# ConwayBeyond/Funscript-Flow

Hardware: AMD Instinct MI355X
Metric: 1080p frame-pairs/sec (higher is better)
Workload: dtype f32

## Files before the change

funscript_flow_amd/csrc/ffl_api.hip:

```cpp
#include "../../include/ffl.h"
#include "ffl_kernels.h"

#include <math.h>
#include <stdarg.h>
#include <stdio.h>
#include <string.h>

#include <algorithm>
#include <condition_variable>
#include <mutex>
#include <string>
#include <thread>
#include <vector>

#define FFL_EV_RING 16
#define FFL_RAW_RING 4

template <class H, class Arg, hipError_t (*Free)(Arg)>
struct Owned {
    H h = H();
    Owned() = default;
    explicit Owned(H take) : h(take) {}
    Owned(Owned &&o) noexcept : h(o.release()) {}
    Owned &operator=(Owned &&o) noexcept { std::swap(h, o.h); return *this; }
// ... 27 lines not shown
    hipError_t create(int n) {
        ev = std::vector<Event>(n);
        for (auto &e : ev) {
            hipError_t r = hipEventCreateWithFlags(e.put(), hipEventDisableTiming);
            if (r != hipSuccess) return r;
        }
        return hipSuccess;
    }
    hipError_t settle_next() {
        if (next < ev.size() || next < settled) return hipSuccess;
        const hipError_t r = hipEventSynchronize(ev[next % ev.size()]);
        if (r == hipSuccess) settled = next + 1;
        return r;
    }
    hipError_t record(hipStream_t st, EvRef *out);
};
struct EvRef {
    const EvRing *ring = nullptr;
    unsigned long long ticket = 0;
    hipEvent_t get() const { return (ring && ring->next - ticket <= ring->ev.size()) ? ring->ev[ticket % ring->ev.size()].h : nullptr; }
};
inline hipError_t EvRing::record(hipStream_t st, EvRef *out) {
    hipError_t r = settle_next();
    if (r == hipSuccess) r = hipEventRecord(ev[next % ev.size()], st);
    if (r == hipSuccess) *out = EvRef{this, next++};
    return r;
}
static inline EvRef ev_latest(const EvRing &r) { return r.next ? EvRef{&r, r.next - 1} : EvRef{}; }

struct ProfRec {
    int cls;
    hipEvent_t a, b;
    bool shared_start;
};

struct LevelGeom {
    int lw, lh, ksize;
    double sigma;
    GaussKernel gk;
};
struct Geometry { int levels = 0; LevelGeom lv[8]; };

struct Layout {
    size_t i_off[8], t_off[8], r_off[8];
    size_t I, T, R;
    size_t M, flow;
    size_t p1, tab;
    size_t gray, bgr;
    size_t slots, res;
};

struct CopyPool {
    struct Job {
        uint8_t *dst;
        const uint8_t *const *srcs;
        size_t row_bytes, dst_frame;
        ptrdiff_t src_pitch;
        int rows, g0, g1;
    };
    std::vector<std::thread> workers;
    std::mutex mu;
    std::condition_variable cv_work, cv_done;
    std::vector<Job> jobs;
    std::vector<char> busy;
    bool stop = false;

// ... 322 lines not shown
    level_geometry(w, h, &geo);
    const size_t N = (size_t)w * h, maxU = 2 * (size_t)max_batch;
    Layout l = {};
    for (int k = 0; k <= geo.levels; k++) {
        const size_t plane = (size_t)geo.lv[k].lw * geo.lv[k].lh;
        l.i_off[k] = l.I; l.t_off[k] = l.T; l.r_off[k] = l.R;
        l.I += plane * maxU;
        l.T += ffl_pyr_tmp_floats(w, h, geo.lv[k].lw) * maxU;
        l.R += 5 * plane * maxU;
    }
    l.M = 5 * N * max_batch; l.flow = 2 * N * max_batch;
    l.p1 = (size_t)ffl_pass1_blocks(w, h) * max_batch; l.tab = FFL_EV_RING;
    l.gray = (size_t)n_frame_slots * N; l.bgr = (size_t)n_frame_slots * N * 3;
    l.slots = 2 * N * n_flow_slots; l.res = n_flow_slots;
    return l;
}

static hipEvent_t prof_event(ffl_ctx *c) {
    Event e;
    if (c->prof_pool.empty()) {
        hipEventCreate(e.put());
    } else {
        e = std::move(c->prof_pool.back());
        c->prof_pool.pop_back();
    }
    return e.release();
}

struct ProfScope {
    ffl_ctx *c;
    int cls;
    hipEvent_t a = nullptr, b = nullptr;
    bool on, shared = false;
    ProfScope(ffl_ctx *c_, int cls_, hipStream_t st, bool chain = false)
        : c(c_), cls(cls_), on((c_->prof_mask >> cls_) & 1u) {
        if (on) {
            stream = st;
            if (chain && c->prof_last_end && c->prof_last_cls == cls && c->prof_last_stream == st) {
                a = c->prof_last_end;
                shared = true;
            } else {
                a = prof_event(c);
                hipEventRecord(a, st);
            }
        } else {
            c->prof_last_end = nullptr;
        }
    }
    ~ProfScope() {
        if (on) {
            b = prof_event(c);
            hipEventRecord(b, stream);
            c->prof_recs.push_back({cls, a, b, shared});
            c->prof_last_end = b;
            c->prof_last_cls = cls;
            c->prof_last_stream = stream;
        }
    }
    hipStream_t stream = nullptr;
};

static void prof_collect(ffl_ctx *c) {
    for (auto &r : c->prof_recs) {
        float ms = 0;
        hipEventSynchronize(r.b);
        hipEventElapsedTime(&ms, r.a, r.b);
        c->prof_launches[r.cls]++;
        c->prof_ms[r.cls] += ms;
    }
    for (auto &r : c->prof_recs) {
        if (!r.shared_start) c->prof_pool.emplace_back(r.a);
        c->prof_pool.emplace_back(r.b);
    }
    c->prof_recs.clear();
    c->prof_last_end = nullptr;
}

struct WaitOnce {
    hipStream_t st;
    hipEvent_t seen[8];
    int n = 0;
    explicit WaitOnce(hipStream_t s) : st(s) {}
    hipError_t operator()(hipEvent_t e) {
        if (!e) return hipSuccess;
        for (int k = 0; k < n; k++)
            if (seen[k] == e) return hipSuccess;
        if (n < 8) seen[n++] = e;
        return hipStreamWaitEvent(st, e, 0);
    }
};

static int wait_unlocked(ffl_ctx *c, CtxLock &lk, const hipEvent_t *evs, int n) {
    HIPCHK(c, hipSetDevice(c->device));
    lk.unlock();
    hipError_t e = hipSuccess;
    for (int i = 0; i < n && e == hipSuccess; i++)
        if (evs[i]) e = hipEventSynchronize(evs[i]);
    lk.lock();
    if (e != hipSuccess) return set_err(c, FFL_ERR_HIP, "hipEventSynchronize failed: %s", hipGetErrorString(e));
    return FFL_OK;
// ... 685 lines not shown
                                int layout, int depth, int msb_aligned, int rw, int rh, int crop_x, int crop_y,
                                const ffl_source_info *si) {
    return upload_yuv(c, "ffl_upload_frames_yuv16", first, n, (const uint8_t *const *)frames, sw, sh, stride_bytes, layout, 2,
                      depth, msb_aligned != 0, rw, rh, crop_x, crop_y, si);
}

int ffl_upload_frame(ffl_ctx *c, int fslot, const uint8_t *data, int width, int height, int channels,
                     ptrdiff_t stride_bytes) {
    return ffl_upload_frames(c, fslot, 1, &data, width, height, channels, stride_bytes);
}

int ffl_download_frame(ffl_ctx *c, int fslot, uint8_t *dst) {
    if (!c) return FFL_ERR_INVALID;
    CtxLock lk(c->mu);
    if (!dst || fslot < 0 || fslot >= c->n_fslots)
        return set_err(c, FFL_ERR_INVALID, "ffl_download_frame: bad frame slot %d", fslot);
    if (!c->frame_valid[fslot]) return set_err(c, FFL_ERR_STATE, "ffl_download_frame: frame slot %d was never uploaded", fslot);
    HIPCHK(c, hipSetDevice(c->device));
    HIPCHK(c, hipMemcpyAsync(dst, c->d_gray + (size_t)fslot * c->N, c->N, hipMemcpyDeviceToHost, c->s_copy));
    HIPCHK(c, hipStreamSynchronize(c->s_copy));
    return FFL_OK;
}

struct DebugCapture {
    int level, iter;
    float *I0, *I1, *R0, *R1, *M, *flow;
};

static int enqueue_batch(ffl_ctx *c, ffl_ctx::Lane &L, const BatchTab &T, int n, int nU, int pov_mode, const DebugCapture *cap) {
    hipStream_t st = L.st;
    const size_t N = c->N;
    const UTab *ut = &L.d_tab->ut;
    const PairTab *pt = &L.d_tab->pt;
    auto pyr_level = [&](int k, hipStream_t s) { ffl_launch_pyr_level(c->d_gray, N, ut, nU, L.pyr[c->geo.levels - k], s); };
    auto expand_level = [&](int k, hipStream_t s) {
        {
            ProfScope ps(c, FFL_K_PYRAMID, s);
            pyr_level(k, s);
        }
        {
            ProfScope ps(c, FFL_K_POLYEXP, s);
            ffl_launch_polyexp(L.poly[c->geo.levels - k], nU, c->pc, s);
        }
    };
    const int mode = cap ? 0 : c->opt.run_ahead;
    if (mode) {
        for (int k = 0; k < (mode == 2 ? 4 : 1); k++)
            if (!L.st_aux[k]) HIPCHK(c, hipStreamCreateWithFlags(L.st_aux[k].put(), hipStreamNonBlocking));
        HIPCHK(c, hipEventRecord(L.ev_fork, st));
        for (int k = c->geo.levels; k >= 0; k--) {
            hipStream_t sa = L.st_aux[mode == 2 ? k : 0];
            if (mode == 2 || k == c->geo.levels) HIPCHK(c, hipStreamWaitEvent(sa, L.ev_fork, 0));
            expand_level(k, sa);
            HIPCHK(c, hipEventRecord(L.ev_R[k], sa));
        }
        if (mode == 2)
            for (int k = c->geo.levels; k >= 0; k--) HIPCHK(c, hipStreamWaitEvent(st, L.ev_R[k], 0));
    }
    const bool run_ahead = mode == 1;
    bool expanded = mode != 0;
    if (mode == 0 && c->opt.merge_expand) {
        const PyrJob *l0 = &L.pyr[L.n_jobs - 1];
        const bool fuse_l0 = c->opt.fuse_l0_blur && ffl_polyexp_from_gray_ok(*l0);
        const int skip_l0 = fuse_l0 && !cap;
        {
            ProfScope ps(c, FFL_K_PYRAMID, st);
            if (!ffl_launch_pyr_multi(c->d_gray, N, ut, nU, L.pyr, L.n_jobs - skip_l0, c->opt, st))
                for (int k = c->geo.levels; k >= skip_l0; k--) pyr_level(k, st);
        }
        {
            ProfScope ps(c, FFL_K_POLYEXP, st);
            ffl_launch_polyexp_multi(L.poly, L.n_jobs, nU, c->pc, c->d_gray, N, ut, fuse_l0 ? l0 : nullptr, st);
        }
        expanded = true;
    }

    int pw = 0, ph = 0;
    for (int k = c->geo.levels; k >= 0; k--) {
        const LevelGeom &g = c->geo.lv[k];
        const int lw = g.lw, lh = g.lh;
        const size_t plane = (size_t)lw * lh;
        const size_t I_stride = plane, R_stride = 5 * plane, M_stride = 5 * plane;
        float *Rk = L.d_R + c->lay.r_off[k];
        if (pw == 0 && cap)
            for (int i = 0; i < n; i++) HIPCHK(c, hipMemsetAsync(T.pt.flow[k][i], 0, sizeof(float) * 2 * plane, st));
        if (run_ahead) HIPCHK(c, hipStreamWaitEvent(st, L.ev_R[k], 0));
        else if (!expanded) expand_level(k, st);
        int mi = 0;
        const bool fuse_first = c->opt.fuse_first > 0 && !cap && (long)((lw + 63) / 64) * ((lh + 15) / 16) * n >= c->opt.fuse_first;
        if (!fuse_first) {
            ProfScope ps(c, FFL_K_UPDATE_MATRICES, st);
            ffl_launch_update_matrices(Rk, R_stride, plane, pt, k, n, L.d_M[mi], M_stride, lw, lh, pw, ph, pw == 0, cap != nullptr, c->opt, st);
        }
        bool captured = false;
        auto capture = [&]() -> int {
            HIPCHK(c, hipStreamSynchronize(st));
            if (cap->I0) HIPCHK(c, hipMemcpy(cap->I0, L.d_I + c->lay.i_off[k] + (size_t)T.pt.u0[0] * I_stride, sizeof(float) * plane, hipMemcpyDeviceToHost));
            if (cap->I1) HIPCHK(c, hipMemcpy(cap->I1, L.d_I + c->lay.i_off[k] + (size_t)T.pt.u1[0] * I_stride, sizeof(float) * plane, hipMemcpyDeviceToHost));
            if (cap->R0) HIPCHK(c, hipMemcpy(cap->R0, Rk + (size_t)T.pt.u0[0] * R_stride, sizeof(float) * 5 * plane, hipMemcpyDeviceToHost));
            if (cap->R1) HIPCHK(c, hipMemcpy(cap->R1, Rk + (size_t)T.pt.u1[0] * R_stride, sizeof(float) * 5 * plane, hipMemcpyDeviceToHost));
            if (cap->M) HIPCHK(c, hipMemcpy(cap->M, L.d_M[mi], sizeof(float) * 5 * plane, hipMemcpyDeviceToHost));
// ... 1353 lines not shown
```

funscript_flow_amd/csrc/ffl_kernels.h:

```cpp
#pragma once
#include <hip/hip_runtime.h>
#include <limits.h>
#include <stdint.h>

#define FFL_MAXB 256
#define FFL_MAXU (2 * FFL_MAXB)
#define FFL_MAX_LEVELS 4
#define FFL_POLY_N 5
#define FFL_WIN 15
#define FFL_WIN_R 7

struct PolyConsts {
    float g[FFL_POLY_N + 1], xg[FFL_POLY_N + 1], xxg[FFL_POLY_N + 1];
    double gd[FFL_POLY_N + 1], xxgd[FFL_POLY_N + 1];
    double ig11, ig03, ig33, ig55;
};

struct GaussKernel {
    float k[32];
    int ksize;
};

struct UTab {
    int fslot[FFL_MAXU];
// ... 70 lines not shown
    float *tmp, *I;
    size_t tmp_stride, I_stride;
    GaussKernel gk;
};
struct PyrJobs {
    PyrJob j[FFL_MAX_JOBS];
    int n;
};
struct PolyJob {
    const float *I;
    float *R;
    size_t I_stride, R_stride, plane;
    int w, h;
    unsigned gx, gy, first, count;
    int from_gray;
    float gk0, gk1;
};
struct PolyJobs {
    PolyJob j[FFL_MAX_JOBS];
    int n;
};

struct FflOptions {
    int lanes = 2;
    int run_ahead = 0;
    int fuse_first = 10000;
    int merge_expand = 1;
    int use_graph = 1;
    int copy_threads = 4;
    int blur_rows = 0;
    int blur_min_wgs = 3500;
    int tile_order = 0;
    int pyr_coarse = 1;
    int fuse_l0_blur = 1;
    int fb_general = 0;
    int import_fused = 1;
};
struct FflOptionRow {
    const char *name;
    int FflOptions::*member;
    int lo, hi;
    bool flag;
};
inline constexpr FflOptionRow kFflOptionRows[] = {
    {"lanes", &FflOptions::lanes, 1, 4, false},
    {"run_ahead", &FflOptions::run_ahead, 0, 2, false},
    {"fuse_first", &FflOptions::fuse_first, 0, INT_MAX, false},
    {"merge_expand", &FflOptions::merge_expand, INT_MIN, INT_MAX, true},
    {"graph", &FflOptions::use_graph, INT_MIN, INT_MAX, true},
    {"copy_threads", &FflOptions::copy_threads, 1, 16, false},
    {"blur_rows", &FflOptions::blur_rows, 0, 64, false},
    {"blur_min_wgs", &FflOptions::blur_min_wgs, 1, INT_MAX, false},
    {"tile_order", &FflOptions::tile_order, 0, 1, false},
    {"pyr_coarse", &FflOptions::pyr_coarse, INT_MIN, INT_MAX, true},
    {"fuse_l0_blur", &FflOptions::fuse_l0_blur, INT_MIN, INT_MAX, true},
    {"fb_general", &FflOptions::fb_general, 0, 1, false},
    {"import_fused", &FflOptions::import_fused, 0, 1, false},
};

bool ffl_launch_pyr_multi(const uint8_t *gray_base, size_t gray_stride, const UTab *ut, int nU, const PyrJob *levels, int n,
                          const FflOptions &opt, hipStream_t st);
bool ffl_polyexp_from_gray_ok(const PyrJob &l0);
void ffl_launch_polyexp_multi(const PolyJob *levels, int n, int nU, PolyConsts pc, const uint8_t *gray_base, size_t gray_stride,
                              const UTab *ut, const PyrJob *l0, hipStream_t st);
void ffl_launch_frontend(const FrameDesc &d, uint8_t *gray, const FrontParams &p, hipStream_t st);
void ffl_launch_frontend_dev(const FrameDesc *tab, int n, uint8_t *gray_base, size_t N, const FrontParams &p, hipStream_t st);
void ffl_launch_export_flows(const float *flow, const ExportTab &tab, int n, size_t N, char *dst, long long item_stride,
                             int layout, hipStream_t st);
void ffl_launch_import_pass1(const ImportArgs &a, const ExportTab &tab, int n, int dtype, int mode, int w, int h, int pov_mode,
                             int fused, PairTab *pt, unsigned long long *pkey, double *psum, hipStream_t st);
void ffl_launch_gray(const uint8_t *bgr, uint8_t *gray, int n_pixels, hipStream_t st);
size_t ffl_pyr_tmp_floats(int w, int h, int lw);
bool ffl_pyr_level_ok(int w, int h, int lw, int lh, int ksize);
void ffl_launch_pyr_level(const uint8_t *gray_base, size_t gray_stride, const UTab *ut, int nU, const PyrJob &level,
                          hipStream_t st);
void ffl_launch_polyexp(const PolyJob &level, int nU, PolyConsts pc, hipStream_t st);
void ffl_launch_update_matrices(const float *R, size_t R_stride, size_t plane, const PairTab *pt, int level, int nB, float *M,
                                size_t M_stride, int lw, int lh, int pw, int ph, int zero_flow, int store_flow,
                                const FflOptions &opt, hipStream_t st);
void ffl_launch_blur_solve(const float *Min, float *Mout, size_t M_stride, const float *R, size_t R_stride,
                           size_t plane, const PairTab *pt, int level, int nB, int lw, int lh, int update, int store_flow,
                           const FflOptions &opt, hipStream_t st);


void ffl_launch_blur_solve_first(float *Mout, size_t M_stride, const float *R, size_t R_stride, size_t plane,
                                 const PairTab *pt, int level, int nB, int lw, int lh, int pw, int ph, const FflOptions &opt,
                                 hipStream_t st);

#define DIS_MAX_PATCHES 4096
#define DIS_MAX_SCALES 12
struct DisKParams {
    int w, h, finest, coarsest, stride, gd_iters, vr_iters, mean_norm, spatial_prop, stripes;
    float alpha, gamma, delta;
    size_t pair_floats;
    size_t pyr_floats;
    size_t pyr_off[DIS_MAX_SCALES];
    float *dbg;
    int dbg_scale, dbg_stage;
};
void ffl_launch_dis(const UTab *ut, const PairTab *pt, int nB, const uint8_t *gray, size_t gray_stride, float *scratch,
                    const DisKParams &p, hipStream_t st);

int ffl_pass1_blocks(int w, int h);
void ffl_launch_pass1(const PairTab *pt, int nB, int w, int h, int pov_mode, unsigned long long *pkey, double *psum,
                      hipStream_t st);

#define FFL_WINDOW_MAX_RADIUS 32
struct WindowSeq {
// ... 209 lines not shown
```

funscript_flow_amd/csrc/kernels_farneback.hip:

```cpp
#include "ffl_kernels.h"

__global__ __launch_bounds__(256) void k_gray(const uint8_t *__restrict__ bgr, uint8_t *__restrict__ gray, int n) {
    int i4 = (blockIdx.x * 256 + threadIdx.x) * 4;
    if (i4 + 3 < n) {
        const uint32_t *p = reinterpret_cast<const uint32_t *>(bgr + (size_t)i4 * 3);
        uint32_t a = p[0], b = p[1], c = p[2];
        uint32_t px[12] = {a & 255, (a >> 8) & 255, (a >> 16) & 255, a >> 24, b & 255, (b >> 8) & 255,
                           (b >> 16) & 255, b >> 24, c & 255, (c >> 8) & 255, (c >> 16) & 255, c >> 24};
        uint32_t o = 0;
#pragma unroll
        for (int j = 0; j < 4; j++) {
            uint32_t g = (px[j * 3] * 3735u + px[j * 3 + 1] * 19235u + px[j * 3 + 2] * 9798u + 16384u) >> 15;
            o |= g << (8 * j);
        }
        *reinterpret_cast<uint32_t *>(gray + i4) = o;
    } else {
        for (int i = i4; i < n; i++) {
            uint32_t b = bgr[(size_t)i * 3], g = bgr[(size_t)i * 3 + 1], r = bgr[(size_t)i * 3 + 2];
            gray[i] = (uint8_t)((b * 3735u + g * 19235u + r * 9798u + 16384u) >> 15);
        }
    }
}

void ffl_launch_gray(const uint8_t *bgr, uint8_t *gray, int n_pixels, hipStream_t st) {
// ... 132 lines not shown
                v1 = v1 + gk.k[R + j] * (V[c - j].y + V[c + j].y);
            }
            t[qy] = v0 * a0 + (a1 == 0.f ? 0.f : v1) * a1;
        }
    } else {
#pragma unroll
        for (int qy = 0; qy < 2; qy++) {
            if (qy == 1 && b1 == 0.f) break;
            const int cy = qy ? y1 : y0;
            float2 c = col[(size_t)cy * lw];
            float v0 = gk.k[R] * c.x, v1 = gk.k[R] * c.y;
#pragma unroll
            for (int j = 1; j <= R; j++) {
                const float2 m = col[(size_t)ffl_reflect101(cy - j, h) * lw], p = col[(size_t)ffl_reflect101(cy + j, h) * lw];
                v0 = v0 + gk.k[R + j] * (m.x + p.x);
                v1 = v1 + gk.k[R + j] * (m.y + p.y);
            }
            t[qy] = v0 * a0 + (a1 == 0.f ? 0.f : v1) * a1;
        }
    }
    if (dyy < lh) I[(size_t)u * I_stride + (size_t)dy * lw + dx] = t[0] * b0 + t[1] * b1;
}
template <int R>
__global__ __launch_bounds__(256) void k_pyr_v2(const float *__restrict__ tmp, size_t tmp_stride, int w, int h, int lw,
                                                int lh, double sx, double sy, GaussKernel gk, float *__restrict__ I,
                                                size_t I_stride) {
    k_pyr_v2_body<R>(blockIdx.x, blockIdx.y, blockIdx.z, tmp, tmp_stride, w, h, lw, lh, sx, sy, gk, I, I_stride);
}

#ifndef FFL_FR1
#define FFL_FR1 8
#define FFL_FR2 2
#endif
template <int S, int FR, bool ALIGNED>
__device__ __forceinline__ void k_pyr_fused3x4_body(const unsigned bx, const unsigned by, const unsigned bz, const uint8_t *__restrict__ gray_base, size_t gray_stride, const UTab *__restrict__ ut,
                                                      int w, int h, int lw, int lh, GaussKernel gk,
                                                      float *__restrict__ I, size_t I_stride) {
    constexpr int NR = S * FR + 2;
    constexpr int NBY = 4 * S + 2;
    const int dx = 4 * (bx * 256 + threadIdx.x), u = bz;
    if (dx >= lw) return;
    const uint8_t *img = gray_base + (size_t)ut->fslot[u] * gray_stride;
    const int cx = S * dx;
    const bool wide = (ALIGNED || (w & 3) == 0) && cx >= 4 && cx + 4 * S + 4 <= w;
    const float k0 = gk.k[1], k1 = gk.k[2];
    const int dy0 = by * FR;
    float H[NR][4 * S];
#pragma unroll
    for (int j = 0; j < NR; j++) {
        const int sy = ffl_reflect101(min(S * dy0 - 1 + j, h + 1), h);
        const uint8_t *row = img + (size_t)sy * w;
        float b[NBY];
        if (wide) {
            uint32_t wd[S + 2];
            if (S == 1) {
                struct __attribute__((packed, aligned(4))) u3 { uint32_t a, b, c; };
                const u3 t = *reinterpret_cast<const u3 *>(row + cx - 4);
                wd[0] = t.a; wd[1] = t.b; wd[2] = t.c;
            } else {
                struct __attribute__((packed, aligned(4))) u4 { uint32_t a, b, c, d; };
                const u4 t = *reinterpret_cast<const u4 *>(row + cx - 4);
                wd[0] = t.a; wd[1] = t.b; wd[2] = t.c; wd[3] = t.d;
            }
            b[0] = (float)(wd[0] >> 24);
#pragma unroll
            for (int t = 0; t < 4 * S; t++) b[1 + t] = (float)((wd[1 + (t >> 2)] >> (8 * (t & 3))) & 255u);
            b[NBY - 1] = (float)(wd[S + 1] & 255u);
        } else {
#pragma unroll
            for (int t = 0; t < NBY; t++) b[t] = (float)row[ffl_reflect101(cx - 1 + t, w)];
        }
#pragma unroll
        for (int c = 0; c < 4 * S; c++) H[j][c] = ffl_blur3(b[c], b[c + 1], b[c + 2], k0, k1);
    }
#pragma unroll
    for (int o = 0; o < FR; o++) {
        const int dy = dy0 + o;
        if (dy >= lh) break;
        const int c = S * o + 1;
        float out[4];
#pragma unroll
        for (int i = 0; i < 4; i++) {
            if (S == 1) {
                out[i] = ffl_lerp_identity(ffl_blur3(H[c - 1][i], H[c][i], H[c + 1][i], k0, k1));
            } else {
                const float v00 = ffl_blur3(H[c - 1][2 * i], H[c][2 * i], H[c + 1][2 * i], k0, k1);
                const float v01 = ffl_blur3(H[c - 1][2 * i + 1], H[c][2 * i + 1], H[c + 1][2 * i + 1], k0, k1);
                const float v10 = ffl_blur3(H[c][2 * i], H[c + 1][2 * i], H[c + 2][2 * i], k0, k1);
                const float v11 = ffl_blur3(H[c][2 * i + 1], H[c + 1][2 * i + 1], H[c + 2][2 * i + 1], k0, k1);
                const float t0 = v00 * 0.5f + v01 * 0.5f, t1 = v10 * 0.5f + v11 * 0.5f;
                out[i] = t0 * 0.5f + t1 * 0.5f;
            }
        }
        float *dst = I + (size_t)u * I_stride + (size_t)dy * lw + dx;
        if (ALIGNED || dx + 3 < lw) {
            ffl_f4u t;
            t.x = out[0]; t.y = out[1]; t.z = out[2]; t.w = out[3];
            *reinterpret_cast<ffl_f4u *>(dst) = t;
        } else {
#pragma unroll
            for (int i = 0; i < 4; i++)
                if (dx + i < lw) dst[i] = out[i];
        }
    }
}
template <int S, int FR, bool ALIGNED>
__global__ __launch_bounds__(256) void k_pyr_fused3x4(const uint8_t *__restrict__ gray_base, size_t gray_stride, const UTab *__restrict__ ut,
                                                      int w, int h, int lw, int lh, GaussKernel gk,
                                                      float *__restrict__ I, size_t I_stride) {
    k_pyr_fused3x4_body<S, FR, ALIGNED>(blockIdx.x, blockIdx.y, blockIdx.z, gray_base, gray_stride, ut, w, h, lw, lh, gk, I, I_stride);
}

#define PC_TW 128
#define PC_TH 64
#define PC_PW 36
#define PC_PH 76
template <int R, int S>
struct PcLevel {
    static constexpr int NC = PC_TW / S;
    static constexpr int NO = NC * (PC_TH / S);
    static constexpr int HROWS = PC_TH + 2 * R - S + 2;
    static constexpr int HROW0 = S / 2 + 5 - R;
    static constexpr int PITCH = 2 * NC + 2;
    static constexpr int B0 = S / 2 + 7 - R;
    static constexpr int ND = (B0 % 4 + 2 * R + 5) / 4;
    static_assert(HROW0 >= 0 && HROW0 + HROWS <= PC_PH && B0 >= 0 && (NC - 1) * (S / 4) + B0 / 4 + ND <= PC_PW, "tile halo");
};
template <int R, int S>
__device__ __forceinline__ void k_pyr_coarse_h(const uint32_t (*sP)[PC_PW], float (*sH)[PcLevel<R, S>::PITCH], const GaussKernel &gk,
                                               int tid) {
    using L = PcLevel<R, S>;
    constexpr int RSTEP = 256 / L::NC, TRIPS = (L::HROWS + RSTEP - 1) / RSTEP, UNROLL = R == 4 ? 3 : TRIPS;
    constexpr int C = L::B0 % 4 + R;
    const int dl = tid % L::NC, rr = tid / L::NC;
#pragma unroll UNROLL
    for (int k = 0; k < TRIPS; k++) {
        const int ry = rr + RSTEP * k;
// ... 12 lines not shown
            *reinterpret_cast<float2 *>(&sH[ry][2 * dl]) = make_float2(a0, a1);
        }
    }
}
template <int R, int S>
__device__ __forceinline__ void k_pyr_coarse_v(const float (*sH)[PcLevel<R, S>::PITCH], const GaussKernel &gk, int tid, int X0,
                                               int Y0, int w, int h, float *__restrict__ I) {
    using L = PcLevel<R, S>;
    const float a1 = 0.5f, a0 = 1.f - a1, b1 = 0.5f, b0 = 1.f - b1;
    const int lw = w / S, lh = h / S;
#pragma unroll
    for (int k = 0; k < (L::NO + 255) / 256; k++) {
        const int o = tid + 256 * k, el = o / L::NC, dl = o % L::NC;
        if (L::NO % 256 != 0 && o >= L::NO) break;
        const int dx = X0 / S + dl, dy = Y0 / S + el;
        float2 V[2 * R + 2];
#pragma unroll
        for (int j = 0; j < 2 * R + 2; j++) V[j] = *reinterpret_cast<const float2 *>(&sH[S * el + j][2 * dl]);
        float tq[2];
#pragma unroll
        for (int qy = 0; qy < 2; qy++) {
            const int c = R + qy;
            float v0 = gk.k[R] * V[c].x, v1 = gk.k[R] * V[c].y;
#pragma unroll
            for (int j = 1; j <= R; j++) {
                v0 = v0 + gk.k[R + j] * (V[c - j].x + V[c + j].x);
                v1 = v1 + gk.k[R + j] * (V[c - j].y + V[c + j].y);
            }
            tq[qy] = v0 * a0 + v1 * a1;
        }
        if (dx < lw && dy < lh) I[(size_t)dy * lw + dx] = tq[0] * b0 + tq[1] * b1;
    }
}
__global__ __launch_bounds__(256) void k_pyr_coarse(const uint8_t *__restrict__ gray_base, size_t gray_stride,
                                                    const UTab *__restrict__ ut, int w, int h, GaussKernel gk2,
                                                    GaussKernel gk3, float *__restrict__ I2, size_t I2_stride,
                                                    float *__restrict__ I3, size_t I3_stride, int tiles_x, int tiles_y,
                                                    int nU) {
    using L2 = PcLevel<4, 4>;
    using L3 = PcLevel<9, 8>;
    __shared__ __attribute__((aligned(8))) uint32_t sP[PC_PH][PC_PW];
    __shared__ __attribute__((aligned(8))) float sH2[L2::HROWS][L2::PITCH];
    __shared__ __attribute__((aligned(8))) float sH3[L3::HROWS][L3::PITCH];
    const int tid = threadIdx.x;
    const unsigned per = (unsigned)tiles_x * tiles_y;
    unsigned tt;
    if (!ffl_xcd_tile(blockIdx.x, per * nU, tt)) return;
    const int u = tt / per, t = tt - u * per, ty = t / tiles_x, tx = t - ty * tiles_x;
    const int X0 = tx * PC_TW, Y0 = ty * PC_TH;
    const uint8_t *img = gray_base + (size_t)ut->fslot[u] * gray_stride;
    constexpr int PCQ = PC_PW / 4, NLOAD = (PC_PH * PCQ + 255) / 256;
#pragma unroll
    for (int k = 0; k < NLOAD; k++) {
        const int i = tid + 256 * k;
        if (i < PC_PH * PCQ) {
            const int ry = i / PCQ, q = i - ry * PCQ;
            const int gy = ffl_reflect101(Y0 - 6 + ry, h), X = X0 - 8 + 16 * q;
            const uint8_t *row = img + (size_t)gy * w;
            uint32_t v[4];
            ffl_gray16_reflect101(row, X, w, true, v);
            *reinterpret_cast<uint2 *>(&sP[ry][4 * q]) = make_uint2(v[0], v[1]);
            *reinterpret_cast<uint2 *>(&sP[ry][4 * q + 2]) = make_uint2(v[2], v[3]);
        }
    }
    __syncthreads();
    k_pyr_coarse_h<4, 4>(sP, sH2, gk2, tid);
    k_pyr_coarse_h<9, 8>(sP, sH3, gk3, tid);
    __syncthreads();
    k_pyr_coarse_v<4, 4>(sH2, gk2, tid, X0, Y0, w, h, I2 + (size_t)u * I2_stride);
    k_pyr_coarse_v<9, 8>(sH3, gk3, tid, X0, Y0, w, h, I3 + (size_t)u * I3_stride);
}

static bool ffl_pyr_coarse_ok(int w, int h, const PyrJob &l2, const PyrJob &l3) {
    return !((w & 7) || (h & 7) || l2.lw != w / 4 || l2.lh != h / 4 || l3.lw != w / 8 || l3.lh != h / 8 ||
             l2.gk.ksize != 9 || l3.gk.ksize != 19);
}
bool ffl_launch_pyr_coarse(const uint8_t *gray_base, size_t gray_stride, const UTab *ut, int nU, int w, int h,
                           const PyrJob &l2, const PyrJob &l3, hipStream_t st) {
    if (!ffl_pyr_coarse_ok(w, h, l2, l3)) return false;
    const int tiles_x = (w + PC_TW - 1) / PC_TW, tiles_y = (h + PC_TH - 1) / PC_TH;
    hipLaunchKernelGGL(k_pyr_coarse, dim3(ffl_xcd_blocks((unsigned)tiles_x * tiles_y * nU)), dim3(256), 0, st, gray_base,
                       gray_stride, ut, w, h, l2.gk, l3.gk, l2.I, l2.I_stride, l3.I, l3.I_stride, tiles_x, tiles_y, nU);
    return true;
}

__global__ __launch_bounds__(256) void k_pyr_multi(const uint8_t *__restrict__ gray_base, size_t gray_stride, const UTab *__restrict__ ut,
                                                   PyrJobs jobs) {
    int i = 0;
#pragma unroll
    for (int t = 1; t < FFL_MAX_JOBS; t++)
        if (t < jobs.n && blockIdx.x >= jobs.j[t].first) i = t;
    const PyrJob &J = jobs.j[i];
    unsigned t;
    if (!ffl_xcd_tile(blockIdx.x - J.first, J.count, t)) return;
    const unsigned per = J.gx * J.gy;
    const unsigned bz = t / per, r = t - bz * per, by = r / J.gx, bx = r - by * J.gx;
    switch (J.kind) {
        case FFL_PYR_F1: k_pyr_fused3x4_body<1, FFL_FR1, true>(bx, by, bz, gray_base, gray_stride, ut, J.w, J.h, J.lw, J.lh, J.gk, J.I, J.I_stride); break;
        case FFL_PYR_F2: k_pyr_fused3x4_body<2, FFL_FR2, true>(bx, by, bz, gray_base, gray_stride, ut, J.w, J.h, J.lw, J.lh, J.gk, J.I, J.I_stride); break;
        case FFL_PYR_H4: k_pyr_h2_body<4>(bx, by, bz, gray_base, gray_stride, ut, J.w, J.h, J.lw, J.sx, J.gk, J.tmp, J.tmp_stride); break;
        case FFL_PYR_H9: k_pyr_h2_body<9>(bx, by, bz, gray_base, gray_stride, ut, J.w, J.h, J.lw, J.sx, J.gk, J.tmp, J.tmp_stride); break;
        case FFL_PYR_V4: k_pyr_v2_body<4>(bx, by, bz, J.tmp, J.tmp_stride, J.w, J.h, J.lw, J.lh, J.sx, J.sy, J.gk, J.I, J.I_stride); break;
        default: k_pyr_v2_body<9>(bx, by, bz, J.tmp, J.tmp_stride, J.w, J.h, J.lw, J.lh, J.sx, J.sy, J.gk, J.I, J.I_stride); break;
    }
}

struct PyrForm {
    int kind;
    bool aligned;
    bool merged;
    unsigned gx, gy;
    unsigned vx, vy;
};
static PyrForm ffl_pyr_form(int w, int h, int lw, int lh, int ksize) {
    const int r = ksize / 2;
    PyrForm f = {};
    f.aligned = (w & 3) == 0 && (lw & 3) == 0;
    if (r == 1 && lw == w && lh == h) f.kind = FFL_PYR_F1;
    else if (r == 1 && w == 2 * lw && h == 2 * lh) f.kind = FFL_PYR_F2;
    else if (r == 1) f.kind = FFL_PYR_H1;
    else if (lw != w && (r == 4 || r == 9)) f.kind = r == 4 ? FFL_PYR_H4 : FFL_PYR_H9;
    else f.kind = FFL_PYR_NONE;
    f.merged = f.aligned && f.kind != FFL_PYR_H1 && f.kind != FFL_PYR_NONE;
    if (f.kind == FFL_PYR_F1 || f.kind == FFL_PYR_F2) {
        const int fr = f.kind == FFL_PYR_F1 ? FFL_FR1 : FFL_FR2;
        f.gx = ((lw + 3) / 4 + 255) / 256;
        f.gy = (lh + fr - 1) / fr;
    } else if (f.kind != FFL_PYR_NONE) {
        const int rows = ffl_pyr_rows(r);
        f.gx = (lw + 255) / 256;
        f.gy = (h + rows - 1) / rows;
        f.vx = (lw + 63) / 64;
        f.vy = (lh + 3) / 4;
    }
    return f;
}
size_t ffl_pyr_tmp_floats(int w, int h, int lw) { return (size_t)h * lw * (lw != w ? 2 : 1); }
bool ffl_pyr_level_ok(int w, int h, int lw, int lh, int ksize) { return ffl_pyr_form(w, h, lw, lh, ksize).kind != FFL_PYR_NONE; }

bool ffl_launch_pyr_multi(const uint8_t *gray_base, size_t gray_stride, const UTab *__restrict__ ut, int nU, const PyrJob *lv, int n,
                          const FflOptions &opt, hipStream_t st) {
    const int w = lv[0].w, h = lv[0].h;
    PyrJobs A = {}, B = {};
    unsigned ta = 0, tb = 0;
    PyrForm form[FFL_MAX_JOBS];
    for (int i = 0; i < n; i++) {
        form[i] = ffl_pyr_form(w, h, lv[i].lw, lv[i].lh, lv[i].gk.ksize);
        if (!form[i].merged) return false;
    }
    int skip0 = -1, skip1 = -1;
    if (opt.pyr_coarse)
        for (int i = 0; i + 1 < n; i++)
            if (lv[i].gk.ksize == 19 && lv[i + 1].gk.ksize == 9 &&
                ffl_launch_pyr_coarse(gray_base, gray_stride, ut, nU, w, h, lv[i + 1], lv[i], st)) {
                skip0 = i;
                skip1 = i + 1;
                break;
            }
    for (int i = 0; i < n; i++) {
        if (i == skip0 || i == skip1) continue;
        const PyrForm &f = form[i];
        PyrJob J = lv[i];
        J.kind = f.kind;
        J.gx = f.gx;
        J.gy = f.gy;
        if (f.vx) {
            PyrJob V = J;
            V.kind = f.kind + (FFL_PYR_V4 - FFL_PYR_H4);
            V.gx = f.vx;
            V.gy = f.vy;
            V.first = tb;
            V.count = V.gx * V.gy * (unsigned)nU;
            tb += ffl_xcd_blocks(V.count);
            B.j[B.n++] = V;
        }
        J.first = ta;
        J.count = J.gx * J.gy * (unsigned)nU;
        ta += ffl_xcd_blocks(J.count);
        A.j[A.n++] = J;
    }
    if (A.n) hipLaunchKernelGGL(k_pyr_multi, dim3(ta), dim3(256), 0, st, gray_base, gray_stride, ut, A);
    if (B.n) hipLaunchKernelGGL(k_pyr_multi, dim3(tb), dim3(256), 0, st, gray_base, gray_stride, ut, B);
    return true;
}

template <int S, int FR>
static void ffl_launch_pyr_fused(const uint8_t *gray_base, size_t gray_stride, const UTab *ut, int nU, const PyrJob &J,
                                 const PyrForm &f, hipStream_t st) {
    const auto kern = f.aligned ? &k_pyr_fused3x4<S, FR, true> : &k_pyr_fused3x4<S, FR, false>;
    hipLaunchKernelGGL(kern, dim3(f.gx, f.gy, nU), dim3(256), 0, st, gray_base, gray_stride, ut, J.w, J.h, J.lw, J.lh, J.gk, J.I,
                       J.I_stride);
}
template <int R>
static void ffl_launch_pyr_hv(const uint8_t *gray_base, size_t gray_stride, const UTab *ut, int nU, const PyrJob &J,
                              const PyrForm &f, hipStream_t st) {
    hipLaunchKernelGGL(k_pyr_h2<R>, dim3(f.gx, f.gy, nU), dim3(256), 0, st, gray_base, gray_stride, ut, J.w, J.h, J.lw, J.sx,
                       J.gk, J.tmp, J.tmp_stride);
    hipLaunchKernelGGL(k_pyr_v2<R>, dim3(f.vx, f.vy, nU), dim3(256), 0, st, J.tmp, J.tmp_stride, J.w, J.h, J.lw, J.lh, J.sx,
                       J.sy, J.gk, J.I, J.I_stride);
}
void ffl_launch_pyr_level(const uint8_t *gray_base, size_t gray_stride, const UTab *ut, int nU, const PyrJob &J,
                          hipStream_t st) {
    const PyrForm f = ffl_pyr_form(J.w, J.h, J.lw, J.lh, J.gk.ksize);
    switch (f.kind) {
        case FFL_PYR_F1: ffl_launch_pyr_fused<1, FFL_FR1>(gray_base, gray_stride, ut, nU, J, f, st); break;
        case FFL_PYR_F2: ffl_launch_pyr_fused<2, FFL_FR2>(gray_base, gray_stride, ut, nU, J, f, st); break;
        case FFL_PYR_H1: ffl_launch_pyr_hv<1>(gray_base, gray_stride, ut, nU, J, f, st); break;
        case FFL_PYR_H4: ffl_launch_pyr_hv<4>(gray_base, gray_stride, ut, nU, J, f, st); break;
        case FFL_PYR_H9: ffl_launch_pyr_hv<9>(gray_base, gray_stride, ut, nU, J, f, st); break;
        default: break;
    }
}

#ifndef PE_TW
#define PE_TW 64
#define PE_TH 16
#endif
#define PE_N FFL_POLY_N
#define PE_LW (PE_TW + 2 * PE_N)
#define PE_LQ ((PE_LW + 3) / 4)
#define PE_PITCH (4 * PE_LQ)

#define PE_UH (PE_TH + 2 * PE_N + 2)
#define PE_UW (PE_LQ + 1)
__device__ __forceinline__ void k_polyexp_body(const unsigned bx, const unsigned by, const unsigned bz, const float *__restrict__ I, size_t I_stride, float *__restrict__ R,
                                                 size_t R_stride, size_t plane, int w, int h, PolyConsts pc,
                                                 const uint8_t *__restrict__ gimg = nullptr, float gk0 = 0.f, float gk1 = 0.f) {
    __shared__ __attribute__((aligned(16))) float sI[PE_TH + 2 * PE_N][PE_PITCH];
    __shared__ __attribute__((aligned(16))) float sV[3][PE_TH][PE_PITCH];
    const int tid = threadIdx.x;
    const int u = bz;
    const int x0 = bx * PE_TW, y0 = by * PE_TH;
    const float *img = I + (size_t)u * I_stride;

    constexpr int N_IN = (PE_TH + 2 * PE_N) * PE_LQ, N_V = PE_TH * PE_LQ;
    if (gimg) {
        static_assert(PE_TW % 8 == 0 && PE_UW % 4 == 0 && 4 * PE_UW >= PE_PITCH + 4, "u8 tile: 16-byte pieces from x0 - 8 on");
        static_assert(sizeof(uint32_t) * PE_UH * PE_UW <= sizeof(sV[0]) && sizeof(float) * PE_UH * PE_PITCH <= 2 * sizeof(sV[0]),
                      "the u8 tile and its horizontal blur fit the dead sV");
        uint32_t (*sU)[PE_UW] = reinterpret_cast<uint32_t (*)[PE_UW]>(&sV[0][0][0]);
        float (*sH)[PE_PITCH] = reinterpret_cast<float (*)[PE_PITCH]>(&sV[1][0][0]);
        const bool words = (w & 3) == 0;
        if (tid < PE_UH * (PE_UW / 4)) {
            const int r = tid / (PE_UW / 4), q = tid - r * (PE_UW / 4);
// ... 723 lines not shown
```

Baseline: 6314.

## Fuse pyramid level-1 downsample into coarse pyramid kernel using shared tile

Folds the level-1 (scale-2) pyramid blur into the k_pyr_coarse kernel, reading from the shared-memory gray tile it already loads for levels 2 and 3. This removes one separate read of the full-resolution gray image and one job from the multi-level pyramid launch. The fused3x4 lane logic is factored into a reusable helper with tap and store callbacks, and the profiler now counts launches per scope. Risks include extra per-block work and register pressure in the coarse kernel.

```diff
diff --git a/funscript_flow_amd/csrc/ffl_api.hip b/funscript_flow_amd/csrc/ffl_api.hip
--- a/funscript_flow_amd/csrc/ffl_api.hip
+++ b/funscript_flow_amd/csrc/ffl_api.hip
@@ -83,6 +83,7 @@
     int cls;
     hipEvent_t a, b;
     bool shared_start;
+    int launches;
 };
 
 struct LevelGeom {
@@ -471,6 +472,7 @@
     int cls;
     hipEvent_t a = nullptr, b = nullptr;
     bool on, shared = false;
+    int launches = 1;
     ProfScope(ffl_ctx *c_, int cls_, hipStream_t st, bool chain = false)
         : c(c_), cls(cls_), on((c_->prof_mask >> cls_) & 1u) {
         if (on) {
@@ -490,7 +492,7 @@
         if (on) {
             b = prof_event(c);
             hipEventRecord(b, stream);
-            c->prof_recs.push_back({cls, a, b, shared});
+            c->prof_recs.push_back({cls, a, b, shared, launches});
             c->prof_last_end = b;
             c->prof_last_cls = cls;
             c->prof_last_stream = stream;
@@ -504,7 +506,7 @@
         float ms = 0;
         hipEventSynchronize(r.b);
         hipEventElapsedTime(&ms, r.a, r.b);
-        c->prof_launches[r.cls]++;
+        c->prof_launches[r.cls] += r.launches;
         c->prof_ms[r.cls] += ms;
     }
     for (auto &r : c->prof_recs) {
@@ -1256,11 +1258,11 @@
     const size_t N = c->N;
     const UTab *ut = &L.d_tab->ut;
     const PairTab *pt = &L.d_tab->pt;
-    auto pyr_level = [&](int k, hipStream_t s) { ffl_launch_pyr_level(c->d_gray, N, ut, nU, L.pyr[c->geo.levels - k], s); };
+    auto pyr_level = [&](int k, hipStream_t s) { return ffl_launch_pyr_level(c->d_gray, N, ut, nU, L.pyr[c->geo.levels - k], s); };
     auto expand_level = [&](int k, hipStream_t s) {
         {
             ProfScope ps(c, FFL_K_PYRAMID, s);
-            pyr_level(k, s);
+            ps.launches = pyr_level(k, s);
         }
         {
             ProfScope ps(c, FFL_K_POLYEXP, s);
@@ -1289,8 +1291,10 @@
         const int skip_l0 = fuse_l0 && !cap;
         {
             ProfScope ps(c, FFL_K_PYRAMID, st);
-            if (!ffl_launch_pyr_multi(c->d_gray, N, ut, nU, L.pyr, L.n_jobs - skip_l0, c->opt, st))
-                for (int k = c->geo.levels; k >= skip_l0; k--) pyr_level(k, st);
+            if (!ffl_launch_pyr_multi(c->d_gray, N, ut, nU, L.pyr, L.n_jobs - skip_l0, c->opt, st, &ps.launches)) {
+                ps.launches = 0;
+                for (int k = c->geo.levels; k >= skip_l0; k--) ps.launches += pyr_level(k, st);
+            }
         }
         {
             ProfScope ps(c, FFL_K_POLYEXP, st);
diff --git a/funscript_flow_amd/csrc/ffl_kernels.h b/funscript_flow_amd/csrc/ffl_kernels.h
--- a/funscript_flow_amd/csrc/ffl_kernels.h
+++ b/funscript_flow_amd/csrc/ffl_kernels.h
@@ -126,6 +126,7 @@
     int blur_min_wgs = 3500;
     int tile_order = 0;
     int pyr_coarse = 1;
+    int pyr_l1 = 1;
     int fuse_l0_blur = 1;
     int fb_general = 0;
     int import_fused = 1;
@@ -147,13 +148,14 @@
     {"blur_min_wgs", &FflOptions::blur_min_wgs, 1, INT_MAX, false},
     {"tile_order", &FflOptions::tile_order, 0, 1, false},
     {"pyr_coarse", &FflOptions::pyr_coarse, INT_MIN, INT_MAX, true},
+    {"pyr_l1", &FflOptions::pyr_l1, 0, 1, false},
     {"fuse_l0_blur", &FflOptions::fuse_l0_blur, INT_MIN, INT_MAX, true},
     {"fb_general", &FflOptions::fb_general, 0, 1, false},
     {"import_fused", &FflOptions::import_fused, 0, 1, false},
 };
 
 bool ffl_launch_pyr_multi(const uint8_t *gray_base, size_t gray_stride, const UTab *ut, int nU, const PyrJob *levels, int n,
-                          const FflOptions &opt, hipStream_t st);
+                          const FflOptions &opt, hipStream_t st, int *launches);
 bool ffl_polyexp_from_gray_ok(const PyrJob &l0);
 void ffl_launch_polyexp_multi(const PolyJob *levels, int n, int nU, PolyConsts pc, const uint8_t *gray_base, size_t gray_stride,
                               const UTab *ut, const PyrJob *l0, hipStream_t st);
@@ -166,8 +168,8 @@
 void ffl_launch_gray(const uint8_t *bgr, uint8_t *gray, int n_pixels, hipStream_t st);
 size_t ffl_pyr_tmp_floats(int w, int h, int lw);
 bool ffl_pyr_level_ok(int w, int h, int lw, int lh, int ksize);
-void ffl_launch_pyr_level(const uint8_t *gray_base, size_t gray_stride, const UTab *ut, int nU, const PyrJob &level,
-                          hipStream_t st);
+int ffl_launch_pyr_level(const uint8_t *gray_base, size_t gray_stride, const UTab *ut, int nU, const PyrJob &level,
+                         hipStream_t st);
 void ffl_launch_polyexp(const PolyJob &level, int nU, PolyConsts pc, hipStream_t st);
 void ffl_launch_update_matrices(const float *R, size_t R_stride, size_t plane, const PairTab *pt, int level, int nB, float *M,
                                 size_t M_stride, int lw, int lh, int pw, int ph, int zero_flow, int store_flow,
diff --git a/funscript_flow_amd/csrc/kernels_farneback.hip b/funscript_flow_amd/csrc/kernels_farneback.hip
--- a/funscript_flow_amd/csrc/kernels_farneback.hip
+++ b/funscript_flow_amd/csrc/kernels_farneback.hip
@@ -188,51 +188,27 @@
 #define FFL_FR1 8
 #define FFL_FR2 2
 #endif
-template <int S, int FR, bool ALIGNED>
-__device__ __forceinline__ void k_pyr_fused3x4_body(const unsigned bx, const unsigned by, const unsigned bz, const uint8_t *__restrict__ gray_base, size_t gray_stride, const UTab *__restrict__ ut,
-                                                      int w, int h, int lw, int lh, GaussKernel gk,
-                                                      float *__restrict__ I, size_t I_stride) {
+template <int S, int FR, class Taps, class Store>
+__device__ __forceinline__ void ffl_fused3x4_lane(float k0, float k1, int rows, Taps taps, Store store) {
     constexpr int NR = S * FR + 2;
     constexpr int NBY = 4 * S + 2;
-    const int dx = 4 * (bx * 256 + threadIdx.x), u = bz;
-    if (dx >= lw) return;
-    const uint8_t *img = gray_base + (size_t)ut->fslot[u] * gray_stride;
-    const int cx = S * dx;
-    const bool wide = (ALIGNED || (w & 3) == 0) && cx >= 4 && cx + 4 * S + 4 <= w;
-    const float k0 = gk.k[1], k1 = gk.k[2];
-    const int dy0 = by * FR;
     float H[NR][4 * S];
 #pragma unroll
     for (int j = 0; j < NR; j++) {
-        const int sy = ffl_reflect101(min(S * dy0 - 1 + j, h + 1), h);
-        const uint8_t *row = img + (size_t)sy * w;
         float b[NBY];
-        if (wide) {
-            uint32_t wd[S + 2];
-            if (S == 1) {
-                struct __attribute__((packed, aligned(4))) u3 { uint32_t a, b, c; };
-                const u3 t = *reinterpret_cast<const u3 *>(row + cx - 4);
-                wd[0] = t.a; wd[1] = t.b; wd[2] = t.c;
-            } else {
-                struct __attribute__((packed, aligned(4))) u4 { uint32_t a, b, c, d; };
-                const u4 t = *reinterpret_cast<const u4 *>(row + cx - 4);
-                wd[0] = t.a; wd[1] = t.b; wd[2] = t.c; wd[3] = t.d;
-            }
+        uint32_t wd[S + 2];
+        if (taps(j, wd, b)) {
             b[0] = (float)(wd[0] >> 24);
 #pragma unroll
             for (int t = 0; t < 4 * S; t++) b[1 + t] = (float)((wd[1 + (t >> 2)] >> (8 * (t & 3))) & 255u);
             b[NBY - 1] = (float)(wd[S + 1] & 255u);
-        } else {
-#pragma unroll
-            for (int t = 0; t < NBY; t++) b[t] = (float)row[ffl_reflect101(cx - 1 + t, w)];
         }
 #pragma unroll
         for (int c = 0; c < 4 * S; c++) H[j][c] = ffl_blur3(b[c], b[c + 1], b[c + 2], k0, k1);
     }
 #pragma unroll
     for (int o = 0; o < FR; o++) {
-        const int dy = dy0 + o;
-        if (dy >= lh) break;
+        if (o >= rows) break;
         const int c = S * o + 1;
         float out[4];
 #pragma unroll
@@ -248,17 +224,53 @@
                 out[i] = t0 * 0.5f + t1 * 0.5f;
             }
         }
-        float *dst = I + (size_t)u * I_stride + (size_t)dy * lw + dx;
-        if (ALIGNED || dx + 3 < lw) {
-            ffl_f4u t;
-            t.x = out[0]; t.y = out[1]; t.z = out[2]; t.w = out[3];
-            *reinterpret_cast<ffl_f4u *>(dst) = t;
-        } else {
-#pragma unroll
-            for (int i = 0; i < 4; i++)
-                if (dx + i < lw) dst[i] = out[i];
-        }
-    }
+        store(o, out);
+    }
+}
+template <int S, int FR, bool ALIGNED>
+__device__ __forceinline__ void k_pyr_fused3x4_body(const unsigned bx, const unsigned by, const unsigned bz, const uint8_t *__restrict__ gray_base, size_t gray_stride, const UTab *__restrict__ ut,
+                                                      int w, int h, int lw, int lh, GaussKernel gk,
+                                                      float *__restrict__ I, size_t I_stride) {
+    constexpr int NBY = 4 * S + 2;
+    const int dx = 4 * (bx * 256 + threadIdx.x), u = bz;
+    if (dx >= lw) return;
+    const uint8_t *img = gray_base + (size_t)ut->fslot[u] * gray_stride;
+    const int cx = S * dx;
+    const bool wide = (ALIGNED || (w & 3) == 0) && cx >= 4 && cx + 4 * S + 4 <= w;
+    const int dy0 = by * FR;
+    ffl_fused3x4_lane<S, FR>(
+        gk.k[1], gk.k[2], lh - dy0,
+        [&](int j, uint32_t (&wd)[S + 2], float (&b)[NBY]) {
+            const int sy = ffl_reflect101(min(S * dy0 - 1 + j, h + 1), h);
+            const uint8_t *row = img + (size_t)sy * w;
+            if (wide) {
+                if (S == 1) {
+                    struct __attribute__((packed, aligned(4))) u3 { uint32_t a, b, c; };
+                    const u3 t = *reinterpret_cast<const u3 *>(row + cx - 4);
+                    wd[0] = t.a; wd[1] = t.b; wd[2] = t.c;
+                } else {
+                    struct __attribute__((packed, aligned(4))) u4 { uint32_t a, b, c, d; };
+                    const u4 t = *reinterpret_cast<const u4 *>(row + cx - 4);
+                    wd[0] = t.a; wd[1] = t.b; wd[2] = t.c; wd[3] = t.d;
+                }
+            } else {
+#pragma unroll
+                for (int t = 0; t < NBY; t++) b[t] = (float)row[ffl_reflect101(cx - 1 + t, w)];
+            }
+            return wide;
+        },
+        [&](int o, const float (&out)[4]) {
+            float *dst = I + (size_t)u * I_stride + (size_t)(dy0 + o) * lw + dx;
+            if (ALIGNED || dx + 3 < lw) {
+                ffl_f4u t;
+                t.x = out[0]; t.y = out[1]; t.z = out[2]; t.w = out[3];
+                *reinterpret_cast<ffl_f4u *>(dst) = t;
+            } else {
+#pragma unroll
+                for (int i = 0; i < 4; i++)
+                    if (dx + i < lw) dst[i] = out[i];
+            }
+        });
 }
 template <int S, int FR, bool ALIGNED>
 __global__ __launch_bounds__(256) void k_pyr_fused3x4(const uint8_t *__restrict__ gray_base, size_t gray_stride, const UTab *__restrict__ ut,
@@ -337,11 +349,35 @@
         if (dx < lw && dy < lh) I[(size_t)dy * lw + dx] = tq[0] * b0 + tq[1] * b1;
     }
 }
+#define PC_L1_NQ (PC_TW / 8)
+#define PC_L1_FR (PC_TH / 2 / (256 / PC_L1_NQ))
+static_assert(2 * (PC_L1_NQ - 1) + 6 <= PC_PW && 2 * PC_L1_FR * (256 / PC_L1_NQ - 1) + 5 + 2 * PC_L1_FR + 2 <= PC_PH, "tile halo");
+__device__ __forceinline__ void k_pyr_coarse_l1(const uint32_t (*sP)[PC_PW], float k0, float k1, int tid, int X0, int Y0, int w,
+                                                int h, float *__restrict__ I) {
+    const int lx = tid % PC_L1_NQ, ly = tid / PC_L1_NQ;
+    const int lw = w / 2, lh = h / 2, dx = X0 / 2 + 4 * lx, dy0 = Y0 / 2 + PC_L1_FR * ly;
+    if (dx >= lw || dy0 >= lh) return;
+    ffl_fused3x4_lane<2, PC_L1_FR>(
+        k0, k1, lh - dy0,
+        [&](int j, uint32_t (&wd)[4], float (&)[10]) {
+            const uint32_t *p = &sP[2 * PC_L1_FR * ly + 5 + j][2 * lx];
+            const uint2 a = *reinterpret_cast<const uint2 *>(p), b = *reinterpret_cast<const uint2 *>(p + 2),
+                        c = *reinterpret_cast<const uint2 *>(p + 4);
+            wd[0] = a.y; wd[1] = b.x; wd[2] = b.y; wd[3] = c.x;
+            return true;
+        },
+        [&](int o, const float (&out)[4]) {
+            ffl_f4u t;
+            t.x = out[0]; t.y = out[1]; t.z = out[2]; t.w = out[3];
+            *reinterpret_cast<ffl_f4u *>(I + (size_t)(dy0 + o) * lw + dx) = t;
+        });
+}
+template <bool L1>
 __global__ __launch_bounds__(256) void k_pyr_coarse(const uint8_t *__restrict__ gray_base, size_t gray_stride,
                                                     const UTab *__restrict__ ut, int w, int h, GaussKernel gk2,
                                                     GaussKernel gk3, float *__restrict__ I2, size_t I2_stride,
                                                     float *__restrict__ I3, size_t I3_stride, int tiles_x, int tiles_y,
-                                                    int nU) {
+                                                    int nU, float gk1k0, float gk1k1, float *__restrict__ I1, size_t I1_stride) {
     using L2 = PcLevel<4, 4>;
     using L3 = PcLevel<9, 8>;
     __shared__ __attribute__((aligned(8))) uint32_t sP[PC_PH][PC_PW];
@@ -369,6 +405,7 @@
         }
     }
     __syncthreads();
+    if (L1) k_pyr_coarse_l1(sP, gk1k0, gk1k1, tid, X0, Y0, w, h, I1 + (size_t)u * I1_stride);
     k_pyr_coarse_h<4, 4>(sP, sH2, gk2, tid);
     k_pyr_coarse_h<9, 8>(sP, sH3, gk3, tid);
     __syncthreads();
@@ -381,11 +418,13 @@
              l2.gk.ksize != 9 || l3.gk.ksize != 19);
 }
 bool ffl_launch_pyr_coarse(const uint8_t *gray_base, size_t gray_stride, const UTab *ut, int nU, int w, int h,
-                           const PyrJob &l2, const PyrJob &l3, hipStream_t st) {
+                           const PyrJob &l2, const PyrJob &l3, const PyrJob *l1, hipStream_t st) {
     if (!ffl_pyr_coarse_ok(w, h, l2, l3)) return false;
     const int tiles_x = (w + PC_TW - 1) / PC_TW, tiles_y = (h + PC_TH - 1) / PC_TH;
-    hipLaunchKernelGGL(k_pyr_coarse, dim3(ffl_xcd_blocks((unsigned)tiles_x * tiles_y * nU)), dim3(256), 0, st, gray_base,
-                       gray_stride, ut, w, h, l2.gk, l3.gk, l2.I, l2.I_stride, l3.I, l3.I_stride, tiles_x, tiles_y, nU);
+    hipLaunchKernelGGL(l1 ? &k_pyr_coarse<true> : &k_pyr_coarse<false>, dim3(ffl_xcd_blocks((unsigned)tiles_x * tiles_y * nU)),
+                       dim3(256), 0, st, gray_base, gray_stride, ut, w, h, l2.gk, l3.gk, l2.I, l2.I_stride, l3.I, l3.I_stride,
+                       tiles_x, tiles_y, nU, l1 ? l1->gk.k[1] : 0.f, l1 ? l1->gk.k[2] : 0.f, l1 ? l1->I : nullptr,
+                       l1 ? l1->I_stride : (size_t)0);
     return true;
 }
 
@@ -444,7 +483,7 @@
 bool ffl_pyr_level_ok(int w, int h, int lw, int lh, int ksize) { return ffl_pyr_form(w, h, lw, lh, ksize).kind != FFL_PYR_NONE; }
 
 bool ffl_launch_pyr_multi(const uint8_t *gray_base, size_t gray_stride, const UTab *__restrict__ ut, int nU, const PyrJob *lv, int n,
-                          const FflOptions &opt, hipStream_t st) {
+                          const FflOptions &opt, hipStream_t st, int *launches) {
     const int w = lv[0].w, h = lv[0].h;
     PyrJobs A = {}, B = {};
     unsigned ta = 0, tb = 0;
@@ -453,17 +492,20 @@
         form[i] = ffl_pyr_form(w, h, lv[i].lw, lv[i].lh, lv[i].gk.ksize);
         if (!form[i].merged) return false;
     }
-    int skip0 = -1, skip1 = -1;
+    int skip0 = -1, skip1 = -1, skip2 = -1;
     if (opt.pyr_coarse)
         for (int i = 0; i + 1 < n; i++)
-            if (lv[i].gk.ksize == 19 && lv[i + 1].gk.ksize == 9 &&
-                ffl_launch_pyr_coarse(gray_base, gray_stride, ut, nU, w, h, lv[i + 1], lv[i], st)) {
-                skip0 = i;
-                skip1 = i + 1;
-                break;
+            if (lv[i].gk.ksize == 19 && lv[i + 1].gk.ksize == 9) {
+                const bool l1 = opt.pyr_l1 && i + 2 < n && form[i + 2].kind == FFL_PYR_F2 && form[i + 2].aligned;
+                if (ffl_launch_pyr_coarse(gray_base, gray_stride, ut, nU, w, h, lv[i + 1], lv[i], l1 ? &lv[i + 2] : nullptr, st)) {
+                    skip0 = i;
+                    skip1 = i + 1;
+                    if (l1) skip2 = i + 2;
+                    break;
+                }
             }
     for (int i = 0; i < n; i++) {
-        if (i == skip0 || i == skip1) continue;
+        if (i == skip0 || i == skip1 || i == skip2) continue;
         const PyrForm &f = form[i];
         PyrJob J = lv[i];
         J.kind = f.kind;
@@ -486,6 +528,7 @@
     }
     if (A.n) hipLaunchKernelGGL(k_pyr_multi, dim3(ta), dim3(256), 0, st, gray_base, gray_stride, ut, A);
     if (B.n) hipLaunchKernelGGL(k_pyr_multi, dim3(tb), dim3(256), 0, st, gray_base, gray_stride, ut, B);
+    if (launches) *launches = (skip0 >= 0) + (A.n > 0) + (B.n > 0);
     return true;
 }
 
@@ -504,8 +547,8 @@
     hipLaunchKernelGGL(k_pyr_v2<R>, dim3(f.vx, f.vy, nU), dim3(256), 0, st, J.tmp, J.tmp_stride, J.w, J.h, J.lw, J.lh, J.sx,
                        J.sy, J.gk, J.I, J.I_stride);
 }
-void ffl_launch_pyr_level(const uint8_t *gray_base, size_t gray_stride, const UTab *ut, int nU, const PyrJob &J,
-                          hipStream_t st) {
+int ffl_launch_pyr_level(const uint8_t *gray_base, size_t gray_stride, const UTab *ut, int nU, const PyrJob &J,
+                         hipStream_t st) {
     const PyrForm f = ffl_pyr_form(J.w, J.h, J.lw, J.lh, J.gk.ksize);
     switch (f.kind) {
         case FFL_PYR_F1: ffl_launch_pyr_fused<1, FFL_FR1>(gray_base, gray_stride, ut, nU, J, f, st); break;
@@ -513,8 +556,9 @@
         case FFL_PYR_H1: ffl_launch_pyr_hv<1>(gray_base, gray_stride, ut, nU, J, f, st); break;
         case FFL_PYR_H4: ffl_launch_pyr_hv<4>(gray_base, gray_stride, ut, nU, J, f, st); break;
         case FFL_PYR_H9: ffl_launch_pyr_hv<9>(gray_base, gray_stride, ut, nU, J, f, st); break;
-        default: break;
-    }
+        default: return 0;
+    }
+    return f.vx ? 2 : 1;
 }
 
 #ifndef PE_TW
```

Measured after the change: 6362 (median of 6 runs). Within noise of the previous version (+0.8%).
